# dwcoen1234/longfellow-zk

Measured on AMD Instinct MI355X. Metric: FFT field-elems/s (batched FFT 2^20 x 1024 rows, Fp128), higher is better.
Workload: dtype u128 (Fp128 Montgomery, 4 x u32 limbs); 1 GPU; batched FFT 2^20 points x 1024 rows per GPU, Fp128 fftb, in place in HBM; field=Fp128 p=2^128-2^108+1, rows_per_gpu=1024, n=1048576, parallelism=rows sharded x1

## Files before the change

### longfellow-zk_amd/csrc/fft.hip

```cpp
#include <string>
#include <type_traits>

#include "ctx.h"
#include "fp_tile_arith.h"

int lf_lch14_fft_bitsliced(lfgpu_ctx* c, int k, int inverse, size_t rows, unsigned l, u64 coset, void* d_B, size_t ld);

#define TILE_ELTS 8192u

struct TilePlan {
  const elt_t* src;
  elt_t* dst;
  long long src_row, dst_row;
  long long src_tile, dst_tile;
  long long sk, sc, dk, dc;
  u32 logT, logC, nbatch;
  u32 kfast_src, kfast_dst;
  u32 wlds;
};

__device__ __forceinline__ u32 bitrev(u32 x, u32 bits) { return bits ? (__brev(x) >> (32 - bits)) : 0; }

__device__ __forceinline__ u32 lds_slot(u32 k, u32 c, u32 logT, u32 logC) {
  u32 slot = (k << logC) + c;
// ... 90 lines not shown
    for (u32 i = tid; i < (T >> 1); i += FFT_THREADS) st16(&wl[i], ld16(&W[(size_t)i << wshift]));
  const u32 wsh = WLDS ? 0 : wshift;
  __syncthreads();
  u32 st = 0;
  while (st < p.logT) {
    const u32 rem = p.logT - st;
    const u32 R = (rem == 3 || rem > 4) ? 3 : (rem >= 2 ? 2 : 1);
    if (WLDS) {
      if (R == 3) fp_radix_round<O, 3, FFT_THREADS>(s, wl, wsh, p.logT, p.logC, st, tid);
      else if (R == 2) fp_radix_round<O, 2, FFT_THREADS>(s, wl, wsh, p.logT, p.logC, st, tid);
      else fp_radix_round<O, 1, FFT_THREADS>(s, wl, wsh, p.logT, p.logC, st, tid);
    } else {
      if (R == 3) fp_radix_round<O, 3, FFT_THREADS>(s, W, wsh, p.logT, p.logC, st, tid);
      else if (R == 2) fp_radix_round<O, 2, FFT_THREADS>(s, W, wsh, p.logT, p.logC, st, tid);
      else fp_radix_round<O, 1, FFT_THREADS>(s, W, wsh, p.logT, p.logC, st, tid);
    }
    __syncthreads();
    st += R;
  }
  for (u32 e = tid; e < T * C; e += FFT_THREADS) {
    u32 j, c;
    if (p.kfast_dst) { j = e & (T - 1); c = e >> p.logT; } else { c = e & (C - 1); j = e >> p.logC; }
    if (cbase + c >= p.nbatch) continue;
    elt_t v = ld16(&s[lds_slot(j, c, p.logT, p.logC)]);
    if (tw_lo) {
      const u32 col = cbase + c, ex = j * col;
      if (ex) {
        if (tw_hi) {
          elt_t t = ld16(&tw_lo[ex & 1023]);
          if (ex >> 10) t = O::mul_tw(t, ld16(&tw_hi[ex >> 10]));
          v = O::mul_tw(v, t);
        } else {
          v = O::mul_tw(v, ld16(&tw_lo[(size_t)j * p.nbatch + col]));
        }
      }
    }
    st16(dst + (long long)j * p.dk + (long long)c * p.dc, v);
  }
}

template <class O>
struct T4Ops : O {
  static __device__ __forceinline__ elt_t add_lazy(elt_t a, elt_t b) { return O::add(a, b); }
  static __device__ __forceinline__ elt_t canon(elt_t a) { return a; }
  static __device__ __forceinline__ elt_t mul_tw_sw(elt_t a, elt_t w) { return O::mul_tw(a, w); }
  static __device__ __forceinline__ void mul2_tw(elt_t& a, elt_t w, elt_t& b, elt_t v) { a = O::mul_tw(a, w), b = O::mul_tw(b, v); }
  static __device__ __forceinline__ void mul2_tw_sw(elt_t& a, elt_t w, elt_t& b, elt_t v) { mul2_tw(a, w, b, v); }
  static __device__ __forceinline__ void canon2(elt_t&, elt_t&) {}
  static __device__ __forceinline__ void bfly_lazy(elt_t& x, elt_t& y) {
    const elt_t u = x, t = y;
    x = O::add(u, t), y = O::sub(u, t);
  }
  static __device__ __forceinline__ void bfly2_lazy(elt_t& xp, elt_t& yp, elt_t& xq, elt_t& yq) { bfly_lazy(xp, yp), bfly_lazy(xq, yq); }
};
#if defined(__HIP_DEVICE_COMPILE__)
template <>
struct T4Ops<Fp128Ops> : Fp128Ops {
  static __device__ __forceinline__ elt_t add(elt_t a, elt_t b) { return fpt_add(a, b); }
  static __device__ __forceinline__ elt_t add_lazy(elt_t a, elt_t b) { return fpt_add_lazy(a, b); }
  static __device__ __forceinline__ elt_t canon(elt_t a) { return fpt_canon(a); }
  static __device__ __forceinline__ elt_t sub(elt_t a, elt_t b) { return fpt_sub(a, b); }
  static __device__ __forceinline__ elt_t mul_tw(elt_t a, elt_t w) { return fpt_mul(a, w); }
  static __device__ __forceinline__ elt_t mul_tw_sw(elt_t a, elt_t w) { return fpt_mul_sw(a, w); }
  static __device__ __forceinline__ void mul2_tw(elt_t& a, elt_t w, elt_t& b, elt_t v) { fpt_mul2(a, w, b, v); }
  static __device__ __forceinline__ void mul2_tw_sw(elt_t& a, elt_t w, elt_t& b, elt_t v) { fpt_mul2_sw(a, w, b, v); }
  static __device__ __forceinline__ void canon2(elt_t& a, elt_t& b) { fpt_canon2(a, b); }
  static __device__ __forceinline__ void bfly_lazy(elt_t& x, elt_t& y) { fpt_bfly_lazy(x, y); }
  static __device__ __forceinline__ void bfly2_lazy(elt_t& xp, elt_t& yp, elt_t& xq, elt_t& yq) { fpt_bfly2_lazy(xp, yp, xq, yq); }
};
#endif
template <class O>
struct T4Ilp : O {};
template <class O>
struct T4IsIlp : std::false_type {};
template <class O>
struct T4IsIlp<T4Ilp<O>> : std::true_type {};
template <class O>
struct T4Ops<T4Ilp<O>> : T4Ops<O> {};

__device__ __forceinline__ u32 t4_slot(u32 p, u32 c, u32 p7) { return ((p << 2) | c) ^ p7; }
__device__ __forceinline__ u32 t4_wslot(u32 i) { return i ^ ((i >> 4) & 15u); }

enum : u32 { T4_CANON = 0, T4_LAZY = 1, T4_LAZY_OUT = 2 };
template <class O, u32 ST, u32 R, bool ROUND0, u32 LZ = T4_CANON>
__device__ __forceinline__ void t4_stages(elt_t* x, u32 j, const elt_t* wl, const elt_t* __restrict__ W, u32 wshift) {
#pragma unroll
  for (u32 t = 0; t < R; ++t) {
    const u32 half = 1u << t;
#pragma unroll
    for (u32 a = 0; a < (1u << R); ++a) {
      if (a & half) continue;
      const u32 jj = j + (a & (half - 1)) * (1u << ST), sh = 9 - ST - t;
      if (!ROUND0) x[a + half] = T4Ops<O>::mul_tw(x[a + half], ld16(&wl[t4_wslot(jj << sh)]));
      else if (a & (half - 1)) x[a + half] = T4Ops<O>::mul_tw(x[a + half], ld16(&W[(size_t)(jj << sh) << wshift]));
      const bool last = LZ == T4_LAZY_OUT && t == R - 1;
      const bool full = LZ == T4_CANON || last || (ROUND0 && ((t == 0 && a != 0) || (t == 1 && a == 4)));
      const elt_t u = last ? T4Ops<O>::canon(x[a]) : x[a], v = x[a + half];
      x[a] = full ? T4Ops<O>::add(u, v) : T4Ops<O>::add_lazy(u, v);
      x[a + half] = T4Ops<O>::sub(u, v);
    }
  }
}

template <class O, u32 LZ>
__device__ __forceinline__ void t4_round0(elt_t* s, const elt_t* y, u32 kb, u32 c, const elt_t* wl, const elt_t* __restrict__ W, u32 wshift) {
  elt_t x[8];
#pragma unroll
  for (u32 a = 0; a < 8; ++a) x[a] = y[((a & 1) << 2) | (a & 2) | (a >> 2)];
  t4_stages<O, 0, 3, true, LZ>(x, 0, wl, W, wshift);
  const u32 b = __brev(kb) >> 25, s0 = t4_slot(8 * b, c, b >> 4), s1 = t4_slot(8 * b + 1, c, b >> 4);
#pragma unroll
  for (u32 a = 0; a < 8; a += 2) {
    st16(&s[s0 + 4 * a], x[a]);
    st16(&s[s1 + 4 * a], x[a + 1]);
  }
}
template <class O, u32 LZ>
__device__ __forceinline__ void t4_round1(elt_t* s, u32 tid, const elt_t* wl, const elt_t* __restrict__ W, u32 wshift) {
  const u32 c = tid & 3, j = (tid >> 2) & 7, h = tid >> 5;
  const u32 s0 = t4_slot(64 * h + j, c, h >> 1);
  elt_t x[8];
// ... 382 lines not shown
    const u32 sk = (u32)p.sk, off = kb * sk + c * (u32)p.sc;
    elt_t y[8], t[8];
#pragma unroll
    for (u32 a = 0; a < 8; ++a) y[a] = ld16(src + (off + 128 * a * sk));
    if (KFAST_SRC) {
      const elt_t* twt = tw + ((size_t)bx << 12);
      const u32 toff = (c << 10) + kb;
#pragma unroll
      for (u32 a = 0; a < 8; ++a) t[a] = ld16(twt + (toff + 128 * a));
    }
    const elt_t wv = ld16(&W[(size_t)tid << wshift]);
#pragma unroll
    for (u32 m = 0; m < 7; ++m) {
      w1[m] = ld16(&W[(size_t)t4w_tw_index<3>(j1, m) << wshift]);
      if (m >= 4) w0[m] = ld16(&W[(size_t)t4w_tw_index<0>(0, m) << wshift]);
    }
#pragma unroll
    for (u32 m = 0; m < 7; ++m) {
      asm volatile("" : "+s"(w1[m].lo), "+s"(w1[m].hi));
      if (m >= 4) asm volatile("" : "+s"(w0[m].lo), "+s"(w0[m].hi));
    }
    w0[2] = w0[5];
    __builtin_amdgcn_sched_barrier(0);
    if (KFAST_SRC) {
      if constexpr (T4IsIlp<O>::value) {
#pragma unroll
        for (u32 a = 0; a < 8; a += 2) T4Ops<O>::mul2_tw(y[a], t[a], y[a + 1], t[a + 1]);
      } else {
#pragma unroll
        for (u32 a = 0; a < 8; ++a) y[a] = T4Ops<O>::mul_tw(y[a], t[a]);
      }
    }
    t4w_round0<O>(s, y, kb, c, w0);
    st16(&wl[t4_wslot(tid)], wv);
  }
  __syncthreads();
  t4w_round1<O>(s, tid, j1, w1);
  __syncthreads();
#pragma unroll
  for (u32 g = 0; g < 2; ++g) t4w_round2<O>(s, tid + 512 * g, wl, W, wshift);
  __syncthreads();
  {
    elt_t* dst = p.dst + (long long)by * p.dst_row + (long long)bx * p.dst_tile;
    const u32 dk = (u32)p.dk, dc = (u32)p.dc;
#pragma unroll
    for (u32 g = 0; g < 2; ++g) {
      const u32 e = tid + 512 * g, c = e & 3, j = e >> 2;
      elt_t x[4];
      t4w_round3_load(x, s, e);
      if constexpr (T4IsIlp<O>::value) t4i_stages4<O, 8, KFAST_SRC ? T4_LAZY_OUT : T4_LAZY>(x, j, wl);
      else t4_stages<O, 8, 2, false, KFAST_SRC ? T4_LAZY_OUT : T4_LAZY>(x, j, wl, W, wshift);
#pragma unroll
      for (u32 a = 0; a < 4; ++a) st16(dst + ((j + 256 * a) * dk + c * dc), x[a]);
    }
  }
}

struct LchTables {
  const elt_t* tbl;
  const elt_t* base;
  u32 nb;
  u32 off[16];
};

template <int FFT_THREADS>
__global__ __launch_bounds__(FFT_THREADS) void lch_fft_tile(TilePlan p, int inverse, LchTables t) {
  extern __shared__ elt_t s[];
  const u32 T = 1u << p.logT, C = 1u << p.logC, tid = threadIdx.x;
  const u32 cbase = blockIdx.x << p.logC;
  const elt_t* src = p.src + (long long)blockIdx.y * p.src_row + (long long)blockIdx.x * p.src_tile;
  elt_t* dst = p.dst + (long long)blockIdx.y * p.dst_row + (long long)blockIdx.x * p.dst_tile;

  for (u32 e = tid; e < T * C; e += FFT_THREADS) {
    u32 k, c;
    if (p.kfast_src) { k = e & (T - 1); c = e >> p.logT; } else { c = e & (C - 1); k = e >> p.logC; }
    elt_t v = elt_zero();
    if (cbase + c < p.nbatch) v = ld16(src + (long long)k * p.sk + (long long)c * p.sc);
    st16(&s[(k << p.logC) + c], v);
  }
  __syncthreads();
  for (u32 step = 0; step < p.logT; ++step) {
    const u32 ii = inverse ? step : (p.logT - 1 - step);
    const u32 sz = 1u << ii;
    for (u32 e = tid; e < (T >> 1) * C; e += FFT_THREADS) {
      u32 c = e & (C - 1), b = e >> p.logC;
      u32 v = b & (sz - 1), u = b >> ii;
      u32 i0 = (u << (ii + 1)) + v, i1 = i0 + sz;
      elt_t tw = ld16(&t.tbl[t.off[ii] + u]);
      if (t.base) {
        u32 cb = cbase + c;
        if (cb >= t.nb) cb = 0;
        tw = gf_add(tw, ld16(&t.base[ii * t.nb + cb]));
      }
      elt_t b0 = ld16(&s[(i0 << p.logC) + c]);
      elt_t b1 = ld16(&s[(i1 << p.logC) + c]);
      if (!inverse) {
        b0 = gf_add(b0, gf_mul(tw, b1));
        b1 = gf_add(b1, b0);
      } else {
        b1 = gf_add(b1, b0);
        b0 = gf_add(b0, gf_mul(tw, b1));
      }
      st16(&s[(i0 << p.logC) + c], b0);
      st16(&s[(i1 << p.logC) + c], b1);
    }
    __syncthreads();
  }
  for (u32 e = tid; e < T * C; e += FFT_THREADS) {
    u32 j, c;
    if (p.kfast_dst) { j = e & (T - 1); c = e >> p.logT; } else { c = e & (C - 1); j = e >> p.logC; }
    if (cbase + c >= p.nbatch) continue;
    st16(dst + (long long)j * p.dk + (long long)c * p.dc, ld16(&s[(j << p.logC) + c]));
  }
}

template <class O>
static int set_lds_limit_fp(lfgpu_ctx* c) {
  LF_HIP(c, hipFuncSetAttribute((const void*)fp_fft_tile<O, 1024, true>, hipFuncAttributeMaxDynamicSharedMemorySize, 160 * 1024));
  LF_HIP(c, hipFuncSetAttribute((const void*)fp_fft_tile<O, 1024, false>, hipFuncAttributeMaxDynamicSharedMemorySize, 160 * 1024));
  LF_HIP(c, hipFuncSetAttribute((const void*)fp_fft_tile<O, 512, true>, hipFuncAttributeMaxDynamicSharedMemorySize, 160 * 1024));
  LF_HIP(c, hipFuncSetAttribute((const void*)fp_fft_tile<O, 512, false>, hipFuncAttributeMaxDynamicSharedMemorySize, 160 * 1024));
  return LFGPU_OK;
}
static int set_lds_limit(lfgpu_ctx* c) {
  if (!(c->attr_done & 1u)) {
    if (const char* e = getenv("LFGPU_TILE_LOG")) {
      int v = atoi(e);
      if (v == 12 || v == 13) c->tile_log = v;
    }
    LF_TRY(set_lds_limit_fp<Fp128Ops>(c));
    const void* const t4[] = {(const void*)fp_fft_tile_1024x4<Fp128Ops, false, true>,
                              (const void*)fp_fft_tile_1024x4<Fp128Ops, true, false>,
                              (const void*)fp_fft_tile_1024x4_persist<Fp128Ops>,
                              (const void*)fp_fft_tile_1024x4_tws<Fp128Ops, false>,
                              (const void*)fp_fft_tile_1024x4_tws<Fp128Ops, true>,
                              (const void*)fp_fft_tile_1024x4_tws_canon<Fp128Ops, false>,
                              (const void*)fp_fft_tile_1024x4_tws_canon<Fp128Ops, true>,
                              (const void*)fp_fft_tile_1024x4_tw2<Fp128Ops, false>,
                              (const void*)fp_fft_tile_1024x4_tw2<Fp128Ops, true>,
                              (const void*)fp_fft_tile_1024x4_tw2<T4Ilp<Fp128Ops>, false>,
                              (const void*)fp_fft_tile_1024x4_tw2<T4Ilp<Fp128Ops>, true>};
    for (const void* k : t4) LF_HIP(c, hipFuncSetAttribute(k, hipFuncAttributeMaxDynamicSharedMemorySize, 160 * 1024));
    LF_TRY(set_lds_limit_fp<F64x2Ops<true>>(c));
    LF_TRY(set_lds_limit_fp<F64x2Ops<false>>(c));
    LF_HIP(c, hipFuncSetAttribute((const void*)lch_fft_tile<1024>, hipFuncAttributeMaxDynamicSharedMemorySize, TILE_ELTS * 16));
    LF_HIP(c, hipFuncSetAttribute((const void*)lch_fft_tile<512>, hipFuncAttributeMaxDynamicSharedMemorySize, TILE_ELTS * 16));
    c->attr_done |= 1u;
  }
  return LFGPU_OK;
}

static size_t fp_lds_bytes(TilePlan& p) {
  const size_t tile = ((size_t)16 << p.logT) << p.logC, tw = (size_t)8 << p.logT;
  p.wlds = tile + tw <= 160u * 1024u ? 1u : 0u;
  return p.wlds ? tile + tw : tile;
}
template <class O, class... Args>
static void launch_fp(lfgpu_ctx* c, dim3 grid, size_t lds, const TilePlan& p, Args... args) {
  if (c->tile_log == 13) {
    if (p.wlds) hipLaunchKernelGGL((fp_fft_tile<O, 1024, true>), grid, dim3(1024), lds, c->stream, p, args...);
    else hipLaunchKernelGGL((fp_fft_tile<O, 1024, false>), grid, dim3(1024), lds, c->stream, p, args...);
  } else {
    if (p.wlds) hipLaunchKernelGGL((fp_fft_tile<O, 512, true>), grid, dim3(512), lds, c->stream, p, args...);
    else hipLaunchKernelGGL((fp_fft_tile<O, 512, false>), grid, dim3(512), lds, c->stream, p, args...);
  }
}
struct FpSwitches {
  bool tile1024;
  int persist;
  int twside;
  bool other_plan;
  bool lazy;
  bool r1wave;
  bool ilp;
  bool two_level;
  bool row_fast;
};
static const FpSwitches& fp_switches() {
  static const FpSwitches sw = [] {
    const auto num = [](const char* name, int dflt) { return getenv(name) ? atoi(getenv(name)) : dflt; };
    FpSwitches w;
    w.tile1024 = num("LFGPU_FP_TILE1024", 1) != 0;
    w.persist = num("LFGPU_FP_PERSIST", 1);
    w.twside = num("LFGPU_FP_TWSIDE", 1);
    w.other_plan = getenv("LFGPU_FP_PERSIST") || getenv("LFGPU_FP_TILE1024");
    w.lazy = num("LFGPU_FP_LAZY", 1) != 0;
    w.r1wave = num("LFGPU_FP_R1WAVE", 1) != 0;
    w.ilp = num("LFGPU_FP_ILP", 1) != 0;
    w.two_level = num("LFGPU_FP_TW", 0) == 2;
    w.row_fast = num("LFGPU_FP_ROWFAST", 1) != 0;
    return w;
  }();
  return sw;
}
static bool tile_1024x4_fits(const TilePlan& p, bool kfast_src, bool offsets32) {
  if (p.logT != 10 || p.logC != 2 || !p.wlds || p.kfast_src != (kfast_src ? 1u : 0u) || p.kfast_dst != 0 || (p.nbatch & 3) != 0) return false;
  return !offsets32 || (p.sk >= 0 && p.sc >= 0 && p.dk >= 0 && p.dc >= 0 && (u64)p.sk * 1024 + (u64)p.sc * 4 <= 0xffffffffu &&
                        (u64)p.dk * 1024 + (u64)p.dc * 4 <= 0xffffffffu);
}
template <class O>
static bool launch_tile_1024x4_persist(lfgpu_ctx* c, u32 rows, size_t lds, const TilePlan& p, const elt_t* W, u32 wshift, const elt_t* tw) {
  const int mode = fp_switches().persist;
  const u32 ncb = p.nbatch >> 2;
  u32 parts = rows;
  if (mode <= 0 || !tile_1024x4_fits(p, false, true)) return false;
  if (mode >= 2) {
    static const int per_cu = [lds] {
      int n = 0;
      if (hipOccupancyMaxActiveBlocksPerMultiprocessor(&n, (const void*)fp_fft_tile_1024x4_persist<O>, 512, lds) != hipSuccess)
        n = 0;
      return n < 1 ? 1 : n;
    }();
    const u32 fill = (u32)per_cu * (u32)c->num_cu;
    parts = fill / ncb;
    if (parts < 1) parts = 1;
    if (parts > rows) parts = rows;
  }
  if ((u64)ncb * parts > 0x7fffffffu) return false;
  const dim3 grid(ncb * parts);
  hipLaunchKernelGGL((fp_fft_tile_1024x4_persist<O>), grid, dim3(512), lds, c->stream, p, W, wshift, tw, rows, parts);
  return true;
}
template <class O, bool KFAST_SRC, bool TW>
static bool launch_tile_1024x4(lfgpu_ctx* c, dim3 grid, size_t lds, const TilePlan& p, const elt_t* W, u32 wshift, const elt_t* tw,
                               u32 row_fast) {
  if constexpr (std::is_same<O, Fp128Ops>::value) {
    if (fp_switches().tile1024 && c->tile_log == 12 && tile_1024x4_fits(p, KFAST_SRC, false)) {
      if constexpr (!KFAST_SRC && TW)
        if (launch_tile_1024x4_persist<O>(c, row_fast ? grid.x : grid.y, lds, p, W, wshift, tw)) return true;
      hipLaunchKernelGGL((fp_fft_tile_1024x4<O, KFAST_SRC, TW>), grid, dim3(512), lds, c->stream, p, W, wshift, tw, row_fast);
      return true;
    }
  }
  return false;
}
template <class O>
static int fp_twside_mode(const lfgpu_ctx* c, u32 logn1, size_t rows, bool two_level) {
  const int mode = fp_switches().other_plan ? 0 : fp_switches().twside;
  if (!std::is_same<O, Fp128Ops>::value || two_level || c->tile_log != 12 || logn1 != 10 || rows > (0x7fffffffu >> 8)) return 0;
  return mode < 0 ? 0 : mode;
}
template <class O, bool KFAST_SRC>
static bool launch_tile_1024x4_tws(lfgpu_ctx* c, u32 rows, size_t lds, const TilePlan& p, const elt_t* W, u32 wshift, const elt_t* tw,
                                   u32 row_fast) {
  if constexpr (std::is_same<O, Fp128Ops>::value) {
    const u32 ncb = p.nbatch >> 2;
    if (!tile_1024x4_fits(p, KFAST_SRC, true) || (u64)ncb * rows > 0x7fffffffu) return false;
    if (KFAST_SRC && (p.sk != 1 || p.sc != 1024 || p.src_tile != 4096)) return false;
    if (KFAST_SRC && (row_fast ? ncb : rows) > 65535) row_fast = !row_fast;
    const dim3 grid = !KFAST_SRC ? dim3(ncb * rows) : row_fast ? dim3(rows, ncb) : dim3(ncb, rows);
    if (!fp_switches().lazy) hipLaunchKernelGGL((fp_fft_tile_1024x4_tws_canon<O, KFAST_SRC>), grid, dim3(512), lds, c->stream, p, W, wshift, tw, row_fast);
    else if (fp_switches().r1wave && fp_switches().ilp) hipLaunchKernelGGL((fp_fft_tile_1024x4_tw2<T4Ilp<O>, KFAST_SRC>), grid, dim3(512), lds, c->stream, p, W, wshift, tw, row_fast);
    else if (fp_switches().r1wave) hipLaunchKernelGGL((fp_fft_tile_1024x4_tw2<O, KFAST_SRC>), grid, dim3(512), lds, c->stream, p, W, wshift, tw, row_fast);
    else hipLaunchKernelGGL((fp_fft_tile_1024x4_tws<O, KFAST_SRC>), grid, dim3(512), lds, c->stream, p, W, wshift, tw, row_fast);
    return true;
  }
  return false;
}
template <class... Args>
static void launch_lch(lfgpu_ctx* c, dim3 grid, size_t lds, Args... args) {
  if (c->tile_log == 13)
    hipLaunchKernelGGL(lch_fft_tile<1024>, grid, dim3(1024), lds, c->stream, args...);
  else
    hipLaunchKernelGGL(lch_fft_tile<512>, grid, dim3(512), lds, c->stream, args...);
}

template <class O>
static elt_t fp_reroot(elt_t w, u64 n, u64 r) {
  while (r < n) {
    w = O::hmul(w, w);
    r += r;
  }
  return w;
}

static std::string keyf(const char* fmt, ...) {
  char buf[256];
  va_list ap;
  va_start(ap, fmt);
  vsnprintf(buf, sizeof(buf), fmt, ap);
  va_end(ap);
  return std::string(buf);
}

static TilePlan plan_single(const lfgpu_ctx* c, void* A, size_t rows, u32 logn, size_t ld) {
  TilePlan p{};
  u32 logC = (u32)c->tile_log - logn;
  u32 need = lf_log2(rows);
  if (logC > need) logC = need;
  p.src = (const elt_t*)A;
  p.dst = (elt_t*)A;
  p.src_row = p.dst_row = 0;
  p.src_tile = p.dst_tile = (long long)ld << logC;
  p.sk = p.dk = 1;
  p.sc = p.dc = (long long)ld;
  p.logT = logn;
  p.logC = logC;
  p.nbatch = (u32)rows;
  p.kfast_src = p.kfast_dst = 1;
  return p;
}

template <class O>
static int fp_root_table(lfgpu_ctx* c, const elt_t wn, u32 logn, u32 logTw, std::string* key_out, void** dW) {
// ... 340 lines not shown
```

### longfellow-zk_amd/csrc/fp_tile_arith.h

```cpp
#pragma once
#include "fields.h"

#if defined(__HIP_DEVICE_COMPILE__)
__device__ __forceinline__ elt_t fpt_add(elt_t a, elt_t b) {
  FP_W(a, a0, a1, a2, a3);
  FP_W(b, b0, b1, b2, b3);
  u32 s0, s1, s2, s3, d0, d1, d2, d3;
  u64 c;
  asm("v_add_co_u32 %0, vcc, %9, %13\n\t"
      "s_nop 1\n\t"
      "v_addc_co_u32 %1, vcc, %10, %14, vcc\n\t"
      "s_nop 1\n\t"
      "v_addc_co_u32 %2, vcc, %11, %15, vcc\n\t"
      "s_nop 1\n\t"
      "v_addc_co_u32 %3, %8, %12, %16, vcc\n\t"
      "v_subrev_co_u32 %4, vcc, 1, %0\n\t"
      "s_nop 1\n\t"
      "v_subbrev_co_u32 %5, vcc, 0, %1, vcc\n\t"
      "s_nop 1\n\t"
      "v_subbrev_co_u32 %6, vcc, 0, %2, vcc\n\t"
      "s_nop 1\n\t"
      "v_subb_co_u32 %7, vcc, %3, %17, vcc\n\t"
      "s_nop 1\n\t"
      "s_andn2_b64 vcc, vcc, %8\n\t"
// ... 171 lines not shown
__device__ __forceinline__ elt_t fpt_mul_sw(elt_t a, elt_t b) { return fpt_mul_t<true>(a, b); }


__device__ __forceinline__ void fpt_bfly2_lazy(elt_t& xp, elt_t& yp, elt_t& xq, elt_t& yq) {
  FP_W(xp, up0, up1, up2, up3);
  FP_W(yp, tp0, tp1, tp2, tp3);
  FP_W(xq, uq0, uq1, uq2, uq3);
  FP_W(yq, tq0, tq1, tq2, tq3);
  u32 dp0, dp1, dp2, dp3, dq0, dq1, dq2, dq3, eap, esp, eaq, esq;
  u64 c1, c2, c3;
  asm("v_add_co_u32 %[dp0], vcc, %[up0], %[tp0]\n\t"
      "v_sub_co_u32 %[tp0], %[c1], %[up0], %[tp0]\n\t"
      "v_add_co_u32 %[dq0], %[c2], %[uq0], %[tq0]\n\t"
      "v_sub_co_u32 %[tq0], %[c3], %[uq0], %[tq0]\n\t"
      "v_addc_co_u32 %[dp1], vcc, %[up1], %[tp1], vcc\n\t"
      "v_subb_co_u32 %[tp1], %[c1], %[up1], %[tp1], %[c1]\n\t"
      "v_addc_co_u32 %[dq1], %[c2], %[uq1], %[tq1], %[c2]\n\t"
      "v_subb_co_u32 %[tq1], %[c3], %[uq1], %[tq1], %[c3]\n\t"
      "v_addc_co_u32 %[dp2], vcc, %[up2], %[tp2], vcc\n\t"
      "v_subb_co_u32 %[tp2], %[c1], %[up2], %[tp2], %[c1]\n\t"
      "v_addc_co_u32 %[dq2], %[c2], %[uq2], %[tq2], %[c2]\n\t"
      "v_subb_co_u32 %[tq2], %[c3], %[uq2], %[tq2], %[c3]\n\t"
      "v_addc_co_u32 %[dp3], vcc, %[up3], %[tp3], vcc\n\t"
      "v_subb_co_u32 %[tp3], %[c1], %[up3], %[tp3], %[c1]\n\t"
      "v_addc_co_u32 %[dq3], %[c2], %[uq3], %[tq3], %[c2]\n\t"
      "v_subb_co_u32 %[tq3], %[c3], %[uq3], %[tq3], %[c3]\n\t"
      "v_cndmask_b32 %[eap], 0, %[k], vcc\n\t"
      "v_cndmask_b32 %[esp], 0, %[k], %[c1]\n\t"
      "v_cndmask_b32 %[eaq], 0, %[k], %[c2]\n\t"
      "v_cndmask_b32 %[esq], 0, %[k], %[c3]\n\t"
      "v_subbrev_co_u32 %[dp0], vcc, 0, %[dp0], vcc\n\t"
      "v_addc_co_u32 %[tp0], %[c1], 0, %[tp0], %[c1]\n\t"
      "v_subbrev_co_u32 %[dq0], %[c2], 0, %[dq0], %[c2]\n\t"
      "v_addc_co_u32 %[tq0], %[c3], 0, %[tq0], %[c3]\n\t"
      "v_subbrev_co_u32 %[dp1], vcc, 0, %[dp1], vcc\n\t"
      "v_addc_co_u32 %[tp1], %[c1], 0, %[tp1], %[c1]\n\t"
      "v_subbrev_co_u32 %[dq1], %[c2], 0, %[dq1], %[c2]\n\t"
      "v_addc_co_u32 %[tq1], %[c3], 0, %[tq1], %[c3]\n\t"
      "v_subbrev_co_u32 %[dp2], vcc, 0, %[dp2], vcc\n\t"
      "v_addc_co_u32 %[tp2], %[c1], 0, %[tp2], %[c1]\n\t"
      "v_subbrev_co_u32 %[dq2], %[c2], 0, %[dq2], %[c2]\n\t"
      "v_addc_co_u32 %[tq2], %[c3], 0, %[tq2], %[c3]\n\t"
      "v_subb_co_u32 %[dp3], vcc, %[dp3], %[eap], vcc\n\t"
      "v_addc_co_u32 %[tp3], %[c1], %[esp], %[tp3], %[c1]\n\t"
      "v_subb_co_u32 %[dq3], %[c2], %[dq3], %[eaq], %[c2]\n\t"
      "v_addc_co_u32 %[tq3], %[c3], %[esq], %[tq3], %[c3]"
      : [dp0] "=&v"(dp0), [dp1] "=&v"(dp1), [dp2] "=&v"(dp2), [dp3] "=&v"(dp3), [dq0] "=&v"(dq0), [dq1] "=&v"(dq1), [dq2] "=&v"(dq2),
        [dq3] "=&v"(dq3), [tp0] "+v"(tp0), [tp1] "+v"(tp1), [tp2] "+v"(tp2), [tp3] "+v"(tp3), [tq0] "+v"(tq0), [tq1] "+v"(tq1),
        [tq2] "+v"(tq2), [tq3] "+v"(tq3), [eap] "=&v"(eap), [esp] "=&v"(esp), [eaq] "=&v"(eaq), [esq] "=&v"(esq), [c1] "=&s"(c1),
        [c2] "=&s"(c2), [c3] "=&s"(c3)
      : [up0] "v"(up0), [up1] "v"(up1), [up2] "v"(up2), [up3] "v"(up3), [uq0] "v"(uq0), [uq1] "v"(uq1), [uq2] "v"(uq2), [uq3] "v"(uq3),
        [k] "v"(0xfffff000u)
      : "vcc");
  xp = FP_PACK(dp0, dp1, dp2, dp3);
  yp = FP_PACK(tp0, tp1, tp2, tp3);
  xq = FP_PACK(dq0, dq1, dq2, dq3);
  yq = FP_PACK(tq0, tq1, tq2, tq3);
}

__device__ __forceinline__ void fpt_bfly_lazy(elt_t& x, elt_t& y) {
  FP_W(x, u0, u1, u2, u3);
  FP_W(y, t0, t1, t2, t3);
  u32 d0, d1, d2, d3, y0, y1, y2, y3, ea, es;
  u64 c1;
  asm("v_add_co_u32 %[d0], vcc, %[u0], %[t0]\n\t"
      "v_sub_co_u32 %[y0], %[c1], %[u0], %[t0]\n\t"
      "s_nop 0\n\t"
      "v_addc_co_u32 %[d1], vcc, %[u1], %[t1], vcc\n\t"
      "v_subb_co_u32 %[y1], %[c1], %[u1], %[t1], %[c1]\n\t"
      "s_nop 0\n\t"
      "v_addc_co_u32 %[d2], vcc, %[u2], %[t2], vcc\n\t"
      "v_subb_co_u32 %[y2], %[c1], %[u2], %[t2], %[c1]\n\t"
      "s_nop 0\n\t"
      "v_addc_co_u32 %[d3], vcc, %[u3], %[t3], vcc\n\t"
      "v_subb_co_u32 %[y3], %[c1], %[u3], %[t3], %[c1]\n\t"
      "s_nop 0\n\t"
      "v_cndmask_b32 %[ea], 0, %[k], vcc\n\t"
      "v_cndmask_b32 %[es], 0, %[k], %[c1]\n\t"
      "v_subbrev_co_u32 %[d0], vcc, 0, %[d0], vcc\n\t"
      "v_addc_co_u32 %[y0], %[c1], 0, %[y0], %[c1]\n\t"
      "s_nop 0\n\t"
      "v_subbrev_co_u32 %[d1], vcc, 0, %[d1], vcc\n\t"
      "v_addc_co_u32 %[y1], %[c1], 0, %[y1], %[c1]\n\t"
      "s_nop 0\n\t"
      "v_subbrev_co_u32 %[d2], vcc, 0, %[d2], vcc\n\t"
      "v_addc_co_u32 %[y2], %[c1], 0, %[y2], %[c1]\n\t"
      "s_nop 0\n\t"
      "v_subb_co_u32 %[d3], vcc, %[d3], %[ea], vcc\n\t"
      "v_addc_co_u32 %[y3], %[c1], %[es], %[y3], %[c1]"
      : [d0] "=&v"(d0), [d1] "=&v"(d1), [d2] "=&v"(d2), [d3] "=&v"(d3), [y0] "=&v"(y0), [y1] "=&v"(y1), [y2] "=&v"(y2), [y3] "=&v"(y3),
        [ea] "=&v"(ea), [es] "=&v"(es), [c1] "=&s"(c1)
      : [u0] "v"(u0), [u1] "v"(u1), [u2] "v"(u2), [u3] "v"(u3), [t0] "v"(t0), [t1] "v"(t1), [t2] "v"(t2), [t3] "v"(t3), [k] "v"(0xfffff000u)
      : "vcc");
  x = FP_PACK(d0, d1, d2, d3);
  y = FP_PACK(y0, y1, y2, y3);
}

__device__ __forceinline__ void fpt_canon2(elt_t& p, elt_t& q) {
  FP_W(p, a0, a1, a2, a3);
  FP_W(q, b0, b1, b2, b3);
  u32 d0, d1, d2, d3, e0, e1, e2, e3;
  u64 c1;
  asm("v_subrev_co_u32 %[d0], vcc, 1, %[a0]\n\t"
      "v_subrev_co_u32 %[e0], %[c1], 1, %[b0]\n\t"
      "s_nop 0\n\t"
      "v_subbrev_co_u32 %[d1], vcc, 0, %[a1], vcc\n\t"
// ... 157 lines not shown
      "v_addc_co_u32 %[pd3], %[pcy], %[pd3], %[pt3], vcc\n\t"
      "v_addc_co_u32 %[qd3], %[qcy], %[qd3], %[qt3], %[qs]\n\t"
      "s_nop 0\n\t"
      "s_andn2_b64 %[pcy], %[pb], %[pcy]\n\t"
      "s_andn2_b64 %[qcy], %[qb], %[qcy]\n\t"
      "v_addc_co_u32 %[pd0], vcc, 0, %[pd0], %[pcy]\n\t"
      "v_addc_co_u32 %[qd0], %[qs], 0, %[qd0], %[qcy]\n\t"
      "v_cndmask_b32 %[pe], 0, %[k], %[pcy]\n\t"
      "v_cndmask_b32 %[qe], 0, %[k], %[qcy]\n\t"
      "v_addc_co_u32 %[pd1], vcc, 0, %[pd1], vcc\n\t"
      "v_addc_co_u32 %[qd1], %[qs], 0, %[qd1], %[qs]\n\t"
      "s_nop 0\n\t"
      "v_addc_co_u32 %[pd2], vcc, 0, %[pd2], vcc\n\t"
      "v_addc_co_u32 %[qd2], %[qs], 0, %[qd2], %[qs]\n\t"
      "s_nop 0\n\t"
      "v_addc_co_u32 %[pd3], vcc, %[pe], %[pd3], vcc\n\t"
      "v_addc_co_u32 %[qd3], %[qs], %[qe], %[qd3], %[qs]"
      : [pd0] "=&v"(pd0), [pd1] "=&v"(pd1), [pd2] "=&v"(pd2), [pd3] "=&v"(pd3), [qd0] "=&v"(qd0), [qd1] "=&v"(qd1), [qd2] "=&v"(qd2),
        [qd3] "=&v"(qd3), [pt0] "+v"(pt0), [pt1] "+v"(pt1), [pt2] "+v"(pt2), [pt3] "+v"(pt3), [qt0] "+v"(qt0), [qt1] "+v"(qt1),
        [qt2] "+v"(qt2), [qt3] "+v"(qt3), [pe] "=&v"(pe), [qe] "=&v"(qe), [pcy] "=&s"(pcy), [pb] "=&s"(pb), [qcy] "=&s"(qcy),
        [qb] "=&s"(qb), [qs] "=&s"(qs)
      : [pk] "v"(pk), [qk] "v"(qk), [k] "v"(0xfffff000u), [pt4] "v"(pt4), [pt5] "v"(pt5), [pt6] "v"(pt6), [pt7] "v"(pt7), [qt4] "v"(qt4),
        [qt5] "v"(qt5), [qt6] "v"(qt6), [qt7] "v"(qt7)
      : "vcc", "scc");
  pa = FP_PACK(pd0, pd1, pd2, pd3);
  qa = FP_PACK(qd0, qd1, qd2, qd3);
}
__device__ __forceinline__ void fpt_mul2(elt_t& pa, elt_t pw, elt_t& qa, elt_t qw) { fpt_mul2_t<false>(pa, pw, qa, qw); }
__device__ __forceinline__ void fpt_mul2_sw(elt_t& pa, elt_t pw, elt_t& qa, elt_t qw) { fpt_mul2_t<true>(pa, pw, qa, qw); }
#else
LF_HD elt_t fpt_add(elt_t a, elt_t b) { return fp_add_c(a, b); }
LF_HD elt_t fpt_sub(elt_t a, elt_t b) { return fp_sub_c(a, b); }
LF_HD elt_t fpt_canon(elt_t a) { return fp_canon128(a); }
LF_HD elt_t fpt_add_lazy(elt_t a, elt_t b) {
  const u64 lo = a.lo + b.lo, c0 = lo < a.lo, h0 = a.hi + b.hi, hi = h0 + c0;
  if (!((h0 < a.hi) | (hi < c0))) return elt_t{lo, hi};
  return elt_t{lo - FP_P_LO, hi - FP_P_HI - (lo < FP_P_LO)};
}
LF_HD elt_t fpt_mul(elt_t a, elt_t b) { return fp_mul_c(fp_canon128(a), b); }
LF_HD elt_t fpt_mul_sw(elt_t a, elt_t b) { return fpt_mul(a, b); }
LF_HD void fpt_bfly_lazy(elt_t& x, elt_t& y) {
  const elt_t u = x, t = y;
  x = fpt_add_lazy(u, t);
  y = fpt_sub(u, t);
}
LF_HD void fpt_bfly2_lazy(elt_t& xp, elt_t& yp, elt_t& xq, elt_t& yq) {
  fpt_bfly_lazy(xp, yp);
  fpt_bfly_lazy(xq, yq);
}
LF_HD void fpt_canon2(elt_t& p, elt_t& q) {
  p = fpt_canon(p);
  q = fpt_canon(q);
}
LF_HD void fpt_mul2(elt_t& pa, elt_t pw, elt_t& qa, elt_t qw) {
  pa = fpt_mul(pa, pw);
  qa = fpt_mul(qa, qw);
}
LF_HD void fpt_mul2_sw(elt_t& pa, elt_t pw, elt_t& qa, elt_t qw) { fpt_mul2(pa, pw, qa, qw); }
#endif
```

Baseline: 48.51 billion field-elems/s.

## Add lean 1024x4 FFT tile kernel with fixed LDS layout and occupancy bounds

New measurement: 49.19 billion field-elems/s (median of 6 runs). 1.4% higher.

```diff
diff --git a/longfellow-zk_amd/csrc/fft.hip b/longfellow-zk_amd/csrc/fft.hip
--- a/longfellow-zk_amd/csrc/fft.hip
+++ b/longfellow-zk_amd/csrc/fft.hip
@@ -166,6 +166,7 @@
     x = O::add(u, t), y = O::sub(u, t);
   }
   static __device__ __forceinline__ void bfly2_lazy(elt_t& xp, elt_t& yp, elt_t& xq, elt_t& yq) { bfly_lazy(xp, yp), bfly_lazy(xq, yq); }
+  static __device__ __forceinline__ void bfly2_full(elt_t& xp, elt_t& yp, elt_t& xq, elt_t& yq) { bfly_lazy(xp, yp), bfly_lazy(xq, yq); }
 };
 #if defined(__HIP_DEVICE_COMPILE__)
 template <>
@@ -181,6 +182,7 @@
   static __device__ __forceinline__ void canon2(elt_t& a, elt_t& b) { fpt_canon2(a, b); }
   static __device__ __forceinline__ void bfly_lazy(elt_t& x, elt_t& y) { fpt_bfly_lazy(x, y); }
   static __device__ __forceinline__ void bfly2_lazy(elt_t& xp, elt_t& yp, elt_t& xq, elt_t& yq) { fpt_bfly2_lazy(xp, yp, xq, yq); }
+  static __device__ __forceinline__ void bfly2_full(elt_t& xp, elt_t& yp, elt_t& xq, elt_t& yq) { fpt_bfly2_full(xp, yp, xq, yq); }
 };
 #endif
 template <class O>
@@ -669,6 +671,201 @@
       else t4_stages<O, 8, 2, false, KFAST_SRC ? T4_LAZY_OUT : T4_LAZY>(x, j, wl, W, wshift);
 #pragma unroll
       for (u32 a = 0; a < 4; ++a) st16(dst + ((j + 256 * a) * dk + c * dc), x[a]);
+    }
+  }
+}
+
+__device__ __forceinline__ u32 t4l_byte(u32 p, u32 c) { return ((p << 6) | (c << 4)) ^ ((p >> 3) & 0x70u) ^ (p & 0xc0u); }
+enum : u32 { T4L_W = 65536, T4L_W8 = T4L_W + 8192, T4L_LDS = T4L_W8 + 1024 };
+typedef u32 t4l_v4 __attribute__((ext_vector_type(4)));
+typedef __attribute__((address_space(3))) t4l_v4 t4l_lds_t;
+__device__ __forceinline__ elt_t t4l_ld(u32 byte) {
+  const t4l_v4 v = *(const t4l_lds_t*)(uintptr_t)byte;
+  return elt_t{((u64)v.y << 32) | v.x, ((u64)v.w << 32) | v.z};
+}
+__device__ __forceinline__ void t4l_st(u32 byte, elt_t e) {
+  const t4l_v4 v = {(u32)e.lo, (u32)(e.lo >> 32), (u32)e.hi, (u32)(e.hi >> 32)};
+  *(t4l_lds_t*)(uintptr_t)byte = v;
+}
+typedef __attribute__((address_space(1))) t4l_v4 t4l_glb_t;
+__device__ __forceinline__ t4l_glb_t* t4l_at(const char* base, u32 step, u32 off) {
+  u64 b = (u64)base + step;
+  asm("" : "+s"(b));
+  return (t4l_glb_t*)(b + off);
+}
+__device__ __forceinline__ elt_t t4l_gld(const t4l_glb_t* q) {
+  const t4l_v4 v = *q;
+  return elt_t{((u64)v.y << 32) | v.x, ((u64)v.w << 32) | v.z};
+}
+__device__ __forceinline__ void t4l_gst(t4l_glb_t* q, elt_t e) {
+  const t4l_v4 v = {(u32)e.lo, (u32)(e.lo >> 32), (u32)e.hi, (u32)(e.hi >> 32)};
+  *q = v;
+}
+template <class O, u32 MODE, u32 T>
+__device__ __forceinline__ void t4l_stage(elt_t* x, const elt_t* w) {
+  constexpr T4iStage S = t4i_plan<MODE>(T);
+  constexpr u32 half = 1u << T, first = half - 1;
+#pragma unroll
+  for (u32 i = 0; i + 1 < S.np; i += 2) {
+    const u32 a = S.prod[i], b = S.prod[i + 1];
+    T4Ops<O>::mul2_tw_sw(x[a + half], w[first + (a & first)], x[b + half], w[first + (b & first)]);
+  }
+  if constexpr (S.np & 1) x[S.prod[S.np - 1] + half] = T4Ops<O>::mul_tw_sw(x[S.prod[S.np - 1] + half], w[first + (S.prod[S.np - 1] & first)]);
+#pragma unroll
+  for (u32 i = 0; i + 1 < S.nc; i += 2) T4Ops<O>::canon2(x[S.can[i] + half], x[S.can[i + 1] + half]);
+  if constexpr (S.nc & 1) x[S.can[S.nc - 1] + half] = T4Ops<O>::canon(x[S.can[S.nc - 1] + half]);
+#pragma unroll
+  for (u32 i = 0; i + 1 < S.nf; i += 2) T4Ops<O>::bfly2_full(x[S.full[i]], x[S.full[i] + half], x[S.full[i + 1]], x[S.full[i + 1] + half]);
+  if constexpr (S.nf & 1) {
+    const u32 a = S.full[S.nf - 1];
+    const elt_t u = x[a], v = x[a + half];
+    x[a] = T4Ops<O>::add(u, v);
+    x[a + half] = T4Ops<O>::sub(u, v);
+  }
+#pragma unroll
+  for (u32 i = 0; i + 1 < S.nl; i += 2) T4Ops<O>::bfly2_lazy(x[S.lazy[i]], x[S.lazy[i] + half], x[S.lazy[i + 1]], x[S.lazy[i + 1] + half]);
+  if constexpr (S.nl & 1) T4Ops<O>::bfly_lazy(x[S.lazy[S.nl - 1]], x[S.lazy[S.nl - 1] + half]);
+}
+template <class O, u32 MODE>
+__device__ __forceinline__ void t4l_stages(elt_t* x, const elt_t* w) {
+  t4l_stage<O, MODE, 0>(x, w);
+  t4l_stage<O, MODE, 1>(x, w);
+  t4l_stage<O, MODE, 2>(x, w);
+}
+template <class O, u32 LZ>
+__device__ __forceinline__ void t4l_stages4(elt_t* x, elt_t w2, elt_t w1, elt_t w1h) {
+  T4Ops<O>::mul2_tw(x[1], w2, x[3], w2);
+  T4Ops<O>::bfly2_lazy(x[0], x[1], x[2], x[3]);
+  T4Ops<O>::mul2_tw(x[2], w1, x[3], w1h);
+  if (LZ == T4_LAZY_OUT) {
+    T4Ops<O>::canon2(x[0], x[1]);
+    T4Ops<O>::bfly2_full(x[0], x[2], x[1], x[3]);
+  } else {
+    T4Ops<O>::bfly2_lazy(x[0], x[2], x[1], x[3]);
+  }
+}
+template <class O>
+__device__ __forceinline__ void t4l_round0(const elt_t* y, u32 kb, u32 c, const elt_t* w) {
+  elt_t x[8];
+#pragma unroll
+  for (u32 a = 0; a < 8; ++a) x[a] = y[((a & 1) << 2) | (a & 2) | (a >> 2)];
+  t4l_stages<O, T4W_R0>(x, w);
+  const u32 s0 = t4l_byte((__brev(kb) >> 25) << 3, c);
+#pragma unroll
+  for (u32 a = 0; a < 8; ++a) t4l_st((s0 ^ (64 * (a & 3))) + 256 * (a >> 2), x[a]);
+}
+template <class O, u32 MODE>
+__device__ __forceinline__ void t4l_round1_wave(u32 s0, const elt_t* w) {
+  elt_t x[8];
+#pragma unroll
+  for (u32 a = 0; a < 8; ++a) x[a] = t4l_ld(s0 + 512 * a);
+  t4l_stages<O, MODE>(x, w);
+#pragma unroll
+  for (u32 a = 0; a < 8; ++a) t4l_st(s0 + 512 * a, x[a]);
+}
+template <class O>
+__device__ __forceinline__ void t4l_round1(u32 tid, u32 j, const elt_t* w, elt_t w8) {
+  const u32 s0 = t4l_byte(((tid >> 2) & 15) << 6, tid & 3) ^ (j << 6);
+  if (j == 0) {
+    t4l_st(T4L_W8 + (tid << 4), w8);
+    asm volatile("; round 1, j = 0");
+    t4l_round1_wave<O, T4W_R1_J0>(s0, w);
+    asm volatile("; round 1, j = 0: stored");
+  } else {
+    asm volatile("; round 1, j > 0");
+    t4l_round1_wave<O, T4W_R1>(s0, w);
+    asm volatile("; round 1, j > 0: stored");
+  }
+}
+template <class O>
+__device__ __forceinline__ void t4l_round2(u32 tid) {
+  const u32 j = (tid >> 2) & 63, s0 = t4l_byte(((tid >> 8) << 8) | j, tid & 3);
+  const u32 sa[4] = {s0, s0 ^ 64, s0 ^ 144, s0 ^ 208};
+  const u32 j16 = (tid << 2) & 0x3f0u;
+  u32 wa = T4L_W8 + j16, wb = T4L_W + 4 * j16;
+  asm("" : "+v"(wa), "+v"(wb));
+  const elt_t w2 = t4l_ld(wa), w1 = t4l_ld(wb), w1h = t4l_ld(wb + 4096);
+#pragma unroll
+  for (u32 g = 0; g < 2; ++g) {
+    elt_t x[4];
+#pragma unroll
+    for (u32 a = 0; a < 4; ++a) x[a] = t4l_ld(sa[a ^ g] + 4096 * a + 32768 * g);
+    t4l_stages4<O, T4_LAZY>(x, w2, w1, w1h);
+#pragma unroll
+    for (u32 a = 0; a < 4; ++a) t4l_st(sa[a ^ g] + 4096 * a + 32768 * g, x[a]);
+  }
+}
+
+template <class O, bool KFAST_SRC>
+__global__ __launch_bounds__(512, 4) void fp_fft_tile_1024x4_lean(TilePlan p, const elt_t* __restrict__ W, u32 wshift,
+                                                                  const elt_t* __restrict__ tw, u32 row_fast, u32 lcb) {
+  const u32 tid = threadIdx.x, j1 = __builtin_amdgcn_readfirstlane(tid >> 6);
+  u32 bx, by;
+  if (KFAST_SRC) {
+    bx = row_fast ? blockIdx.y : blockIdx.x;
+    by = row_fast ? blockIdx.x : blockIdx.y;
+  } else {
+    const u32 i = blockIdx.x >> 3, sh = lcb - 3;
+    bx = ((blockIdx.x & 7) << sh) + (i & ((1u << sh) - 1));
+    by = i >> sh;
+  }
+  elt_t w0[7] = {}, w1[7], wv8;
+  {
+    const u32 c = KFAST_SRC ? tid >> 7 : tid & 3, kb = KFAST_SRC ? tid & 127 : tid >> 2;
+    const char* src = (const char*)(p.src + (long long)by * p.src_row + (long long)bx * p.src_tile);
+    const u32 sk = (u32)p.sk << 4, off = kb * sk + c * ((u32)p.sc << 4);
+    elt_t y[8], t[8];
+#pragma unroll
+    for (u32 a = 0; a < 8; ++a) y[a] = t4l_gld(t4l_at(src, 128 * a * sk, off));
+    if (KFAST_SRC) {
+      const char* twt = (const char*)(tw + ((size_t)bx << 12));
+      const u32 toff = ((c << 10) + kb) << 4;
+#pragma unroll
+      for (u32 a = 0; a < 8; ++a) t[a] = t4l_gld(t4l_at(twt, 2048 * a, toff));
+    }
+    const elt_t wv = t4l_gld(t4l_at((const char*)W, 0, tid << (wshift + 4)));
+    wv8 = t4l_gld(t4l_at((const char*)W, 0, (tid & 63) << (wshift + 7)));
+#pragma unroll
+    for (u32 m = 0; m < 7; ++m) {
+      w1[m] = ld16(&W[(size_t)t4w_tw_index<3>(j1, m) << wshift]);
+      if (m >= 4) w0[m] = ld16(&W[(size_t)t4w_tw_index<0>(0, m) << wshift]);
+    }
+#pragma unroll
+    for (u32 m = 0; m < 7; ++m) {
+      asm volatile("" : "+s"(w1[m].lo), "+s"(w1[m].hi));
+      if (m >= 4) asm volatile("" : "+s"(w0[m].lo), "+s"(w0[m].hi));
+    }
+    w0[2] = w0[5];
+    __builtin_amdgcn_sched_barrier(0);
+    if (KFAST_SRC) {
+#pragma unroll
+      for (u32 a = 0; a < 8; a += 2) T4Ops<O>::mul2_tw(y[a], t[a], y[a + 1], t[a + 1]);
+    }
+    t4l_round0<O>(y, kb, c, w0);
+    asm volatile("" ::"v"(wv8.lo), "v"(wv8.hi));
+    t4l_st(T4L_W + (tid << 4), wv);
+  }
+  __syncthreads();
+  t4l_round1<O>(tid, j1, w1, wv8);
+  __syncthreads();
+  t4l_round2<O>(tid);
+  __syncthreads();
+  {
+    char* dst = (char*)(p.dst + (long long)by * p.dst_row + (long long)bx * p.dst_tile);
+    const u32 j0 = tid >> 2, c = tid & 3, dk = (u32)p.dk << 4, off = j0 * dk + c * ((u32)p.dc << 4);
+    const u32 s0 = t4l_byte(j0, c);
+    u32 wa = T4L_W + ((tid << 3) & ~31u), wb = T4L_W + ((tid << 2) & ~15u);
+    asm("" : "+v"(wa), "+v"(wb));
+#pragma unroll
+    for (u32 g = 0; g < 2; ++g) {
+      const u32 sg = g ? s0 ^ 144 : s0;
+      elt_t x[4];
+#pragma unroll
+      for (u32 a = 0; a < 4; ++a) x[a] = t4l_ld((sg ^ (32 * a)) + 16384 * a + 8192 * g);
+      const elt_t w2 = t4l_ld(wa + 4096 * g), w1s = t4l_ld(wb + 2048 * g), w1h = t4l_ld(wb + 2048 * g + 4096);
+      t4l_stages4<O, KFAST_SRC ? T4_LAZY_OUT : T4_LAZY>(x, w2, w1s, w1h);
+#pragma unroll
+      for (u32 a = 0; a < 4; ++a) t4l_gst(t4l_at(dst, (128 * g + 256 * a) * dk, off), x[a]);
     }
   }
 }
@@ -756,7 +953,9 @@
                               (const void*)fp_fft_tile_1024x4_tw2<Fp128Ops, false>,
                               (const void*)fp_fft_tile_1024x4_tw2<Fp128Ops, true>,
                               (const void*)fp_fft_tile_1024x4_tw2<T4Ilp<Fp128Ops>, false>,
-                              (const void*)fp_fft_tile_1024x4_tw2<T4Ilp<Fp128Ops>, true>};
+                              (const void*)fp_fft_tile_1024x4_tw2<T4Ilp<Fp128Ops>, true>,
+                              (const void*)fp_fft_tile_1024x4_lean<T4Ilp<Fp128Ops>, false>,
+                              (const void*)fp_fft_tile_1024x4_lean<T4Ilp<Fp128Ops>, true>};
     for (const void* k : t4) LF_HIP(c, hipFuncSetAttribute(k, hipFuncAttributeMaxDynamicSharedMemorySize, 160 * 1024));
     LF_TRY(set_lds_limit_fp<F64x2Ops<true>>(c));
     LF_TRY(set_lds_limit_fp<F64x2Ops<false>>(c));
@@ -790,6 +989,7 @@
   bool lazy;
   bool r1wave;
   bool ilp;
+  bool lean;
   bool two_level;
   bool row_fast;
 };
@@ -804,6 +1004,7 @@
     w.lazy = num("LFGPU_FP_LAZY", 1) != 0;
     w.r1wave = num("LFGPU_FP_R1WAVE", 1) != 0;
     w.ilp = num("LFGPU_FP_ILP", 1) != 0;
+    w.lean = num("LFGPU_FP_LEAN", 1) != 0;
     w.two_level = num("LFGPU_FP_TW", 0) == 2;
     w.row_fast = num("LFGPU_FP_ROWFAST", 1) != 0;
     return w;
@@ -814,6 +1015,13 @@
   if (p.logT != 10 || p.logC != 2 || !p.wlds || p.kfast_src != (kfast_src ? 1u : 0u) || p.kfast_dst != 0 || (p.nbatch & 3) != 0) return false;
   return !offsets32 || (p.sk >= 0 && p.sc >= 0 && p.dk >= 0 && p.dc >= 0 && (u64)p.sk * 1024 + (u64)p.sc * 4 <= 0xffffffffu &&
                         (u64)p.dk * 1024 + (u64)p.dc * 4 <= 0xffffffffu);
+}
+static bool tile_1024x4_lean_fits(const TilePlan& p, bool kfast_src, u32 wshift, u32* lcb) {
+  const u32 ncb = p.nbatch >> 2;
+  if (ncb == 0 || (ncb & (ncb - 1)) != 0 || (!kfast_src && ncb < 8) || wshift > 16) return false;
+  if (((u64)p.sk * 1024 + (u64)p.sc * 4) * 16 > 0xffffffffu || ((u64)p.dk * 1024 + (u64)p.dc * 4) * 16 > 0xffffffffu) return false;
+  *lcb = lf_log2(ncb);
+  return true;
 }
 template <class O>
 static bool launch_tile_1024x4_persist(lfgpu_ctx* c, u32 rows, size_t lds, const TilePlan& p, const elt_t* W, u32 wshift, const elt_t* tw) {
@@ -866,7 +1074,10 @@
     if (KFAST_SRC && (p.sk != 1 || p.sc != 1024 || p.src_tile != 4096)) return false;
     if (KFAST_SRC && (row_fast ? ncb : rows) > 65535) row_fast = !row_fast;
     const dim3 grid = !KFAST_SRC ? dim3(ncb * rows) : row_fast ? dim3(rows, ncb) : dim3(ncb, rows);
+    u32 lcb = 0;
     if (!fp_switches().lazy) hipLaunchKernelGGL((fp_fft_tile_1024x4_tws_canon<O, KFAST_SRC>), grid, dim3(512), lds, c->stream, p, W, wshift, tw, row_fast);
+    else if (fp_switches().r1wave && fp_switches().ilp && fp_switches().lean && tile_1024x4_lean_fits(p, KFAST_SRC, wshift, &lcb))
+      hipLaunchKernelGGL((fp_fft_tile_1024x4_lean<T4Ilp<O>, KFAST_SRC>), grid, dim3(512), T4L_LDS, c->stream, p, W, wshift, tw, row_fast, lcb);
     else if (fp_switches().r1wave && fp_switches().ilp) hipLaunchKernelGGL((fp_fft_tile_1024x4_tw2<T4Ilp<O>, KFAST_SRC>), grid, dim3(512), lds, c->stream, p, W, wshift, tw, row_fast);
     else if (fp_switches().r1wave) hipLaunchKernelGGL((fp_fft_tile_1024x4_tw2<O, KFAST_SRC>), grid, dim3(512), lds, c->stream, p, W, wshift, tw, row_fast);
     else hipLaunchKernelGGL((fp_fft_tile_1024x4_tws<O, KFAST_SRC>), grid, dim3(512), lds, c->stream, p, W, wshift, tw, row_fast);
diff --git a/longfellow-zk_amd/csrc/fp_tile_arith.h b/longfellow-zk_amd/csrc/fp_tile_arith.h
--- a/longfellow-zk_amd/csrc/fp_tile_arith.h
+++ b/longfellow-zk_amd/csrc/fp_tile_arith.h
@@ -247,6 +247,71 @@
       : [up0] "v"(up0), [up1] "v"(up1), [up2] "v"(up2), [up3] "v"(up3), [uq0] "v"(uq0), [uq1] "v"(uq1), [uq2] "v"(uq2), [uq3] "v"(uq3),
         [k] "v"(0xfffff000u)
       : "vcc");
+  xp = FP_PACK(dp0, dp1, dp2, dp3);
+  yp = FP_PACK(tp0, tp1, tp2, tp3);
+  xq = FP_PACK(dq0, dq1, dq2, dq3);
+  yq = FP_PACK(tq0, tq1, tq2, tq3);
+}
+
+__device__ __forceinline__ void fpt_bfly2_full(elt_t& xp, elt_t& yp, elt_t& xq, elt_t& yq) {
+  FP_W(xp, up0, up1, up2, up3);
+  FP_W(yp, tp0, tp1, tp2, tp3);
+  FP_W(xq, uq0, uq1, uq2, uq3);
+  FP_W(yq, tq0, tq1, tq2, tq3);
+  u32 sp0, sp1, sp2, sp3, sq0, sq1, sq2, sq3, dp0, dp1, dp2, dp3, dq0, dq1, dq2, dq3, ep, eq;
+  u64 ap, aq, sp, sq, bq;
+  asm("v_add_co_u32 %[sp0], %[ap], %[up0], %[tp0]\n\t"
+      "v_sub_co_u32 %[tp0], %[sp], %[up0], %[tp0]\n\t"
+      "v_add_co_u32 %[sq0], %[aq], %[uq0], %[tq0]\n\t"
+      "v_sub_co_u32 %[tq0], %[sq], %[uq0], %[tq0]\n\t"
+      "v_addc_co_u32 %[sp1], %[ap], %[up1], %[tp1], %[ap]\n\t"
+      "v_subb_co_u32 %[tp1], %[sp], %[up1], %[tp1], %[sp]\n\t"
+      "v_addc_co_u32 %[sq1], %[aq], %[uq1], %[tq1], %[aq]\n\t"
+      "v_subb_co_u32 %[tq1], %[sq], %[uq1], %[tq1], %[sq]\n\t"
+      "v_addc_co_u32 %[sp2], %[ap], %[up2], %[tp2], %[ap]\n\t"
+      "v_subb_co_u32 %[tp2], %[sp], %[up2], %[tp2], %[sp]\n\t"
+      "v_addc_co_u32 %[sq2], %[aq], %[uq2], %[tq2], %[aq]\n\t"
+      "v_subb_co_u32 %[tq2], %[sq], %[uq2], %[tq2], %[sq]\n\t"
+      "v_addc_co_u32 %[sp3], %[ap], %[up3], %[tp3], %[ap]\n\t"
+      "v_subb_co_u32 %[tp3], %[sp], %[up3], %[tp3], %[sp]\n\t"
+      "v_addc_co_u32 %[sq3], %[aq], %[uq3], %[tq3], %[aq]\n\t"
+      "v_subb_co_u32 %[tq3], %[sq], %[uq3], %[tq3], %[sq]\n\t"
+      "v_subrev_co_u32 %[dp0], vcc, 1, %[sp0]\n\t"
+      "v_subrev_co_u32 %[dq0], %[bq], 1, %[sq0]\n\t"
+      "v_cndmask_b32 %[ep], 0, %[k], %[sp]\n\t"
+      "v_cndmask_b32 %[eq], 0, %[k], %[sq]\n\t"
+      "v_subbrev_co_u32 %[dp1], vcc, 0, %[sp1], vcc\n\t"
+      "v_subbrev_co_u32 %[dq1], %[bq], 0, %[sq1], %[bq]\n\t"
+      "v_addc_co_u32 %[tp0], %[sp], 0, %[tp0], %[sp]\n\t"
+      "v_addc_co_u32 %[tq0], %[sq], 0, %[tq0], %[sq]\n\t"
+      "v_subbrev_co_u32 %[dp2], vcc, 0, %[sp2], vcc\n\t"
+      "v_subbrev_co_u32 %[dq2], %[bq], 0, %[sq2], %[bq]\n\t"
+      "v_addc_co_u32 %[tp1], %[sp], 0, %[tp1], %[sp]\n\t"
+      "v_addc_co_u32 %[tq1], %[sq], 0, %[tq1], %[sq]\n\t"
+      "v_subb_co_u32 %[dp3], vcc, %[sp3], %[k], vcc\n\t"
+      "v_subb_co_u32 %[dq3], %[bq], %[sq3], %[k], %[bq]\n\t"
+      "v_addc_co_u32 %[tp2], %[sp], 0, %[tp2], %[sp]\n\t"
+      "v_addc_co_u32 %[tq2], %[sq], 0, %[tq2], %[sq]\n\t"
+      "s_andn2_b64 vcc, vcc, %[ap]\n\t"
+      "s_andn2_b64 %[bq], %[bq], %[aq]\n\t"
+      "v_cndmask_b32 %[dp0], %[dp0], %[sp0], vcc\n\t"
+      "v_cndmask_b32 %[dq0], %[dq0], %[sq0], %[bq]\n\t"
+      "v_addc_co_u32 %[tp3], %[sp], %[ep], %[tp3], %[sp]\n\t"
+      "v_addc_co_u32 %[tq3], %[sq], %[eq], %[tq3], %[sq]\n\t"
+      "v_cndmask_b32 %[dp1], %[dp1], %[sp1], vcc\n\t"
+      "v_cndmask_b32 %[dq1], %[dq1], %[sq1], %[bq]\n\t"
+      "v_cndmask_b32 %[dp2], %[dp2], %[sp2], vcc\n\t"
+      "v_cndmask_b32 %[dq2], %[dq2], %[sq2], %[bq]\n\t"
+      "v_cndmask_b32 %[dp3], %[dp3], %[sp3], vcc\n\t"
+      "v_cndmask_b32 %[dq3], %[dq3], %[sq3], %[bq]"
+      : [sp0] "=&v"(sp0), [sp1] "=&v"(sp1), [sp2] "=&v"(sp2), [sp3] "=&v"(sp3), [sq0] "=&v"(sq0), [sq1] "=&v"(sq1), [sq2] "=&v"(sq2),
+        [sq3] "=&v"(sq3), [dp0] "=&v"(dp0), [dp1] "=&v"(dp1), [dp2] "=&v"(dp2), [dp3] "=&v"(dp3), [dq0] "=&v"(dq0), [dq1] "=&v"(dq1),
+        [dq2] "=&v"(dq2), [dq3] "=&v"(dq3), [tp0] "+v"(tp0), [tp1] "+v"(tp1), [tp2] "+v"(tp2), [tp3] "+v"(tp3), [tq0] "+v"(tq0),
+        [tq1] "+v"(tq1), [tq2] "+v"(tq2), [tq3] "+v"(tq3), [ep] "=&v"(ep), [eq] "=&v"(eq), [ap] "=&s"(ap), [aq] "=&s"(aq), [sp] "=&s"(sp),
+        [sq] "=&s"(sq), [bq] "=&s"(bq)
+      : [up0] "v"(up0), [up1] "v"(up1), [up2] "v"(up2), [up3] "v"(up3), [uq0] "v"(uq0), [uq1] "v"(uq1), [uq2] "v"(uq2), [uq3] "v"(uq3),
+        [k] "v"(0xfffff000u)
+      : "vcc", "scc");
   xp = FP_PACK(dp0, dp1, dp2, dp3);
   yp = FP_PACK(tp0, tp1, tp2, tp3);
   xq = FP_PACK(dq0, dq1, dq2, dq3);
@@ -510,6 +575,11 @@
   p = fpt_canon(p);
   q = fpt_canon(q);
 }
+LF_HD void fpt_bfly2_full(elt_t& xp, elt_t& yp, elt_t& xq, elt_t& yq) {
+  const elt_t up = xp, tp = yp, uq = xq, tq = yq;
+  xp = fpt_add(up, tp), yp = fpt_sub(up, tp);
+  xq = fpt_add(uq, tq), yq = fpt_sub(uq, tq);
+}
 LF_HD void fpt_mul2(elt_t& pa, elt_t pw, elt_t& qa, elt_t qw) {
   pa = fpt_mul(pa, pw);
   qa = fpt_mul(qa, qw);
```
